# hermanjakobsen/robotic-ultrasound-imaging

Hardware: AMD Instinct MI355X
Metric: env-steps/sec (whole node) at 4096 envs/GPU, random-action rollout (higher is better)
Workload: dtype f32

## Files before the change

### robotic-ultrasound-imaging_amd/csrc/usim_step16.h

```cpp
#pragma once
#include <type_traits>

namespace usim {

template <int N, class F>
DI void static_for(F&& f) {
    if constexpr (N > 0) { static_for<N - 1>(f); f(std::integral_constant<int, N - 1>{}); }
}

template <int CTRL>
DI float dpp0(float v) { return __int_as_float(__builtin_amdgcn_update_dpp(0, __float_as_int(v), CTRL, 0xf, 0xf, true)); }
template <int G> DI int glane() { return (int)(threadIdx.x & (G - 1)); }
template <int G, int K> DI float rbc(float v) {
    if constexpr (G == 16) return dpp0<0x150 + K>(v);
    else {
        const int iv = __float_as_int(v);
        const int t = __builtin_amdgcn_update_dpp(iv, iv, 0x150 + K, 0xf, 0x3, false);
        return __int_as_float(__builtin_amdgcn_update_dpp(t, iv, 0x150 + 8 + K, 0xf, 0xc, false));
    }
}
template <int G, int D> DI float rshr0(float v) {
    const float t = dpp0<0x110 + D>(v);
    if constexpr (G == 16) return t; else return (glane<G>() < D) ? 0.f : t;
}
// ... 115 lines not shown
    P = mk(at[AT_LPOS], at[AT_LPOS + 1], at[AT_LPOS + 2]);
    static_for<3>([&](auto Dc) {
        constexpr int D = 1 << decltype(Dc)::value;
        const f3 LX = mk(rshr<G, D>(X.x, 1.f), rshr<G, D>(X.y, 0.f), rshr<G, D>(X.z, 0.f));
        const f3 LY = mk(rshr<G, D>(Y.x, 0.f), rshr<G, D>(Y.y, 1.f), rshr<G, D>(Y.z, 0.f));
        const f3 LZ = mk(rshr<G, D>(Z.x, 0.f), rshr<G, D>(Z.y, 0.f), rshr<G, D>(Z.z, 1.f));
        const f3 LP = mk(rshr0<G, D>(P.x), rshr0<G, D>(P.y), rshr0<G, D>(P.z));
        const f3 nX = LX * X.x + LY * X.y + LZ * X.z, nY = LX * Y.x + LY * Y.y + LZ * Y.z, nZ = LX * Z.x + LY * Z.y + LZ * Z.z;
        P = LP + LX * P.x + LY * P.y + LZ * P.z;
        X = nX; Y = nY; Z = nZ;
    });
}

DI void jacobian_rows(float* xl, const int gl, const float* Jc, float* Jr) {
    if (gl < 8) {
#pragma unroll
        for (int a = 0; a < 6; ++a) xl[a * 8 + gl] = Jc[a];
    }
    group_sync();
    int arow = (gl & 7) - ((gl & 4) ? 1 : 0);
    arow = arow > 5 ? 5 : arow;
    const float4 j0 = *reinterpret_cast<const float4*>(&xl[arow * 8]), j1 = *reinterpret_cast<const float4*>(&xl[arow * 8 + 4]);
    Jr[0] = j0.x; Jr[1] = j0.y; Jr[2] = j0.z; Jr[3] = j0.w; Jr[4] = j1.x; Jr[5] = j1.y; Jr[6] = j1.z; Jr[7] = j1.w;
}

template <int G>
DI float solve6_task(float* A, float b, const int gl) {
    static_for<6>([&](auto Kc) {
        constexpr int k = decltype(Kc)::value;
        constexpr int lk = TASK_LANE[k];
        const float g = (A[k] - (gl == lk ? 1.f : 0.f)) * rcp_(rbc<G, lk>(A[k]));
#pragma unroll
        for (int c = k + 1; c < 6; ++c) A[c] = fmaf(-g, rbc<G, lk>(A[c]), A[c]);
        b = fmaf(-g, rbc<G, lk>(b), b);
    });
    return b;
}

constexpr int X16_WORDS = 64;
constexpr int X16_RIGID_STRIDE = 84;

#ifndef USIM_WPR16
#define USIM_WPR16 4
#endif
#ifndef USIM_WPR8
#define USIM_WPR8 4
#endif
template <int G> constexpr int wpr() { return G == 16 ? USIM_WPR16 : USIM_WPR8; }
constexpr int MB_POSE = X16_WORDS;
constexpr int MB_OP = MB_POSE + 12;
constexpr int MB_W = MB_OP + 64;
constexpr int MB_Q = MB_W + 16;
constexpr int MB_GOAL = MB_Q + 100;
constexpr int X2_STRIDE = MB_GOAL + 12;
template <int G> constexpr int x2_base() { return TB_WORDS + (64 * wpr<G>() / G) * GE_STRIDE; }
static_assert(x2_base<16>() % 4 == 0 && x2_base<8>() % 4 == 0 && X2_STRIDE % 4 == 0 && MB_OP % 4 == 0 && MB_W % 4 == 0, "mailbox block: 16-byte accesses");
static_assert((x2_base<8>() + 32 * X2_STRIDE) * 4 <= 160 * 1024, "split kernel with 8-lane groups: LDS of a CU");
template <int G> constexpr int arm_cull_rounds() { return 7; }

#if defined(USIM_TSTAMP) || defined(USIM_TSTAMP_NOWAIT)
#define USIM_BAR() do { __syncthreads(); ++nbar; } while (0)
#else
#define USIM_BAR() __syncthreads()
#endif


constexpr int ARM_LDS_WORDS = A16_LANES * AT_STRIDE;
template <int TORSO, int ROLE, int G> constexpr int arm_lds_base();
template <int NE, class WR = NoWarm>
struct Carry {
    float dqj, qdj, q0j;
    Episode ep;
    float s[NE], sd[NE];
    WR wr;
};

template <int TORSO, int ROLE, int G> constexpr int arm_lds_base() {
    return ROLE != 0 ? x2_base<G>() + (64 * wpr<G>() / G) * X2_STRIDE : (TORSO ? SOFT16_LDS_WORDS : 16 * X16_RIGID_STRIDE);
}
static_assert((arm_lds_base<1, 1, 8>() + ARM_LDS_WORDS) * 4 <= 160 * 1024 && arm_lds_base<1, 1, 8>() % 4 == 0 && arm_lds_base<1, 1, 16>() % 4 == 0 && arm_lds_base<1, 0, 16>() % 4 == 0
              && arm_lds_base<0, 0, 16>() % 4 == 0, "arm table behind the LDS blocks of every 16-lane kernel");

template <int TORSO, int MODE, int ROLE, int NT, int G = 16, bool RES = false, class WR = NoWarm>
DI void step16_one(float* lds, const DevModel& M, const DevCfg& C, float* __restrict__ st, const int n, const int npad, const DevIO& io, const int flags, const long long rstep,
                   const bool first_pass, const int sub, int& nbar, Carry<TORSO ? (N_TOP + G - 1) / G : 1, WR>& cy) {
    constexpr bool WARM = !std::is_same<WR, NoWarm>::value;
    static_assert(!WARM || (TORSO == 1 && ROLE == 0) || (TORSO == 1 && MODE == 0), "warm start: the soft-torso kernels");
    constexpr int WPR = (ROLE != 0) ? wpr<G>() : 4;
    constexpr int EPW = 64 / G, EPB = WPR * EPW;
    static_assert(!RES || MODE == 0, "resident state: step launches only");
    constexpr int X2_BASE = x2_base<G>();
    constexpr unsigned GMASK = (G == 16) ? 0xffffu : 0xffu;
    static_assert(G == 16 || (TORSO == 1 && MODE == 0 && ROLE != 0), "8-lane groups: the split soft-torso step only");
    constexpr int NE = TORSO ? (N_TOP + G - 1) / G : 1;
    static_assert(ROLE == 0 || (TORSO == 1 && MODE == 0), "the split kernel is the soft-torso step");
    const int lane = threadIdx.x & 63, wave = (threadIdx.x >> 6) & (WPR - 1);
    constexpr bool RES_HERE = RES && !(ROLE == 2 && G == 16);
    const bool fresh = !RES_HERE || first_pass;
    const int gl = lane & (G - 1), ge = lane / G;
    const int gbase = lane - gl;
    const int eb = wave * EPW + ge;
    const bool auto_reset = (flags & LF_AUTO_RESET) != 0;
    unsigned long long* const dbg = io.dbg;
    const bool refill = (MODE == 1) && io.refill != 0;
    const int item_cnt = refill ? io.count[0] : 1;
    const int item_first = refill ? (int)blockIdx.x * EPB : 0;
    for (int item0 = item_first; item0 < item_cnt; item0 += refill ? (int)gridDim.x * EPB : 1) {
    int env = blockIdx.x * EPB + eb;
    bool valid = env < n;
    int item_ep = 0;
    if (refill) {
        valid = item0 + eb < item_cnt;
        const int2 it = valid ? io.items[item0 + eb] : make_int2(0, 0);
        env = it.x; item_ep = it.y;
    }
    const bool store = valid && gl == 0;
    const int ei = valid ? env : (refill ? 0 : n - 1);
#define LAT(w) st[(size_t)F_LAT * npad + (size_t)ei * LAT_ENV_WORDS + (w)]
#define EB(off) lds[TB_WORDS + eb * GE_STRIDE + (off)]
    float* const warm_rows = st + warm_index(io.bank_row0, npad, (size_t)ei);
    int mbo = X2_BASE + eb * X2_STRIDE;
    if constexpr (ROLE != 0) asm volatile("" : "+v"(mbo));
    float* const xl = (ROLE != 0) ? &lds[mbo]
                                  : (TORSO ? &lds[TB_WORDS + eb * GE_STRIDE + GE_WS] : &lds[eb * X16_RIGID_STRIDE]);
    static_assert(GE_WS + X16_WORDS <= GE_STRIDE, "transpose scratch overlays the wrench records");
    constexpr int GOAL_OFF = (ROLE != 0) ? MB_GOAL : (TORSO ? GE_CG + (MAXCAND + 1) * CG_WORDS - GE_WS : X16_WORDS);
    static_assert(GE_CG + (MAXCAND + 1) * CG_WORDS + 12 <= GE_STRIDE && X16_WORDS + 12 <= X16_RIGID_STRIDE, "room for the goal");
    float* const goal_lds = xl + GOAL_OFF;

    USIM_STAMP(dbg, 0);
    if constexpr (ROLE == 1) { if (dbg && blockIdx.x == 0 && threadIdx.x == 0) dbg[20] = __builtin_readcyclecounter(); }

    float at[AT_STRIDE];
    {
        constexpr int ARM_LDS = arm_lds_base<TORSO, ROLE, G>();
        const float4* ap = fresh ? reinterpret_cast<const float4*>(M.tables + TB_ARM + gl * AT_STRIDE) : reinterpret_cast<const float4*>(lds + ARM_LDS + gl * AT_STRIDE);
        if (fresh) {
#pragma unroll
            for (int v = 0; v < AT_STRIDE / 4; ++v) { const float4 x = ap[v]; at[4 * v] = x.x; at[4 * v + 1] = x.y; at[4 * v + 2] = x.z; at[4 * v + 3] = x.w; }
            if constexpr (RES && ROLE != 2) {
                if (lane < G) {
#pragma unroll
                    for (int v = 0; v < AT_STRIDE / 4; ++v) reinterpret_cast<float4*>(lds + ARM_LDS + gl * AT_STRIDE)[v] = make_float4(at[4 * v], at[4 * v + 1], at[4 * v + 2], at[4 * v + 3]);
// ... 58 lines not shown
        int tix = threadIdx.x;
        asm volatile("" : "+v"(tix));
#pragma unroll
        for (int i = 0; i < PER; ++i) { int idx = tix + i * NT; tmp[i] = (idx < NV) ? src[idx] : make_float4(0, 0, 0, 0); }
#pragma unroll
        for (int i = 0; i < PER; ++i) { int idx = tix + i * NT; if (idx < NV) dst[idx] = tmp[i]; }
        USIM_BAR();
    }
    USIM_STAMP(dbg, 1);

    if (MODE == 0 && sub == 0) t += 1;
    const bool last_sub = sub == C.substeps - 1;
    const int tphys = (MODE == 0) ? (t - 1) * C.substeps + sub : 0;
    const float dt = C.dt, inv_h = rcp_((float)C.horizon);
#if defined(USIM_TSTAMP) || defined(USIM_TSTAMP_NOWAIT)
#define RSTAMP(k) do { if (dbg && blockIdx.x == 0 && (threadIdx.x & (64 * WPR - 1)) == 0) dbg[(ROLE == 2 ? 30 : 20) + (k)] = __builtin_readcyclecounter(); } while (0)
#else
#define RSTAMP(k) do { } while (0)
#endif
#define XSTAMP(k) RSTAMP(20 + (k))
    if constexpr (ROLE == 2) {
        RSTAMP(0);
        float* const mb = &lds[mbo];
        const int* tb_shell = reinterpret_cast<const int*>(lds + TB_SHELL);
        float dz, vz, az;
        torso_motion(C, tphys, dz, vz, az);
        lattice_rhs<G, NE>(lds, eb, gl, M, az, kst, kdmp, true, s_pre, sd_pre);
        lattice_solve<G>(lds, eb, gl, gbase);
        RSTAMP(1);
        USIM_BAR();
        RSTAMP(2);
        const f3 xs = mk(mb[MB_POSE], mb[MB_POSE + 1], mb[MB_POSE + 2]), sy = mk(mb[MB_POSE + 3], mb[MB_POSE + 4], mb[MB_POSE + 5]),
                 sz = mk(mb[MB_POSE + 6], mb[MB_POSE + 7], mb[MB_POSE + 8]);
        const f3 sxc = cross(sy, sz);
        int nq = __float_as_int(mb[MB_POSE + 10]);
#pragma unroll
        for (int i = arm_cull_rounds<G>(); i < NE; ++i) {
            const int eraw = i * G + gl, e = eraw < N_TOP ? eraw : N_TOP - 1;
            const bool cand = (eraw < N_TOP) && collide_cull(lds, e, M, C, s_pre[i], dz, xs, sxc, sz);
            const unsigned gm = (unsigned)(__ballot(cand) >> gbase) & GMASK;
            mb[MB_Q + (cand ? nq + __popc(gm & ((1u << gl) - 1u)) : 99)] = __int_as_float(e);
            nq += __popc(gm);
        }
        group_sync();
        int nc = 0;
        collide_queue<G>(lds, mb + MB_Q, nq, &EB(GE_CG), gl, gbase, M, C, &EB(GE_S), dz, xs, sxc, sy, sz, nc);
        constexpr bool EARLY = G == 8;
        ContactRows P;
        int nc_early = nc, overflow_early = 0, ncmax_early = 0, cel_early[MAXC];
        if constexpr (EARLY) {
            contact_overflow<G>(lds, eb, gl, gbase, nc_early);
            if (nc_early > MAXC) { overflow_early = 1; nc_early = MAXC; }
            group_sync();
#pragma unroll
            for (int k = MAXC; k >= 1; --k) if (ncmax_early == 0 && __any(nc_early >= k)) ncmax_early = k;
#pragma unroll
            for (int k = 0; k < MAXC; ++k) cel_early[k] = (k < nc_early) ? __float_as_int(EB(GE_CG + k * CG_WORDS + 6)) : 0;
            if (ncmax_early > 0) contact_rows<G>(lds, eb, gl, M, C, nc_early, cel_early, vz, P);
        }
        RSTAMP(3);
        USIM_BAR();
        RSTAMP(4);
        if constexpr (!EARLY) contact_overflow<G>(lds, eb, gl, gbase, nc);
        int overflow = 0;
        if (nc > MAXC) { overflow = 1; nc = MAXC; }
        if constexpr (!EARLY) group_sync();
        XSTAMP(0);
        int ncmax = 0;
        if constexpr (EARLY) { nc = nc_early; overflow = overflow_early; ncmax = ncmax_early; }
        else {
#pragma unroll
            for (int k = MAXC; k >= 1; --k) if (ncmax == 0 && __any(nc >= k)) ncmax = k;
        }
        XSTAMP(1);
        float gf[MAXC], W[6] = {0, 0, 0, 0, 0, 0};
        int cel[MAXC];
#pragma unroll
        for (int k = 0; k < MAXC; ++k) { const int ek = __float_as_int(EB(GE_CG + k * CG_WORDS + 6)); gf[k] = 0.f; cel[k] = EARLY ? cel_early[k] : ((k < nc) ? ek : 0); }
        if (ncmax > 0) {
            float alpha[6], vs[6], Lp[21];
#pragma unroll
            for (int a = 0; a < 6; ++a) {
                alpha[a] = mb[MB_OP + 48 + a]; vs[a] = mb[MB_OP + 54 + a];
#pragma unroll
                for (int b = 0; b <= a; ++b) Lp[PK(a, b)] = mb[MB_OP + a * 8 + b];
            }
            XSTAMP(2);
            contact_solve<G, EARLY, true>(lds, eb, gl, M, C, nc, ncmax, cel, Lp, alpha, vs, mu, vz, P, W, gf, dbg, cy.wr);
            XSTAMP(3);
        } else warm_clear(cy.wr);
        if (gl == 0) {
            *reinterpret_cast<float4*>(&mb[MB_W]) = make_float4(W[0], W[1], W[2], W[3]);
            *reinterpret_cast<float4*>(&mb[MB_W + 4]) = make_float4(W[4], W[5], __int_as_float(nc), __int_as_float(overflow));
#pragma unroll
            for (int k = 0; k < MAXC; ++k) { const int sh = tb_shell[cel[k]]; mb[MB_W + 8 + k] = __int_as_float((k < nc) ? sh : -1); }
        }
        RSTAMP(5);
        USIM_BAR();
        RSTAMP(6);
        {
            float acc_e[NE];
#pragma unroll
            for (int i = 0; i < NE; ++i) { const int e = gl + i * G; acc_e[i] = (e < N_TOP) ? EB(GE_A + e) : 0.f; }
#pragma unroll
            for (int k = 0; k < MAXC; ++k) {
#pragma unroll
                for (int i = 0; i < NE; ++i) {
                    const int e = (gl + i * G < N_TOP) ? gl + i * G : N_TOP - 1;
                    acc_e[i] = fmaf(lds[TB_LINV + e * LROW + cel[k]], gf[k], acc_e[i]);
                }
            }
#pragma unroll
            for (int i = 0; i < NE; ++i) {
                const int e = gl + i * G;
                if (e >= N_TOP) continue;
                const float sdn = sd_pre[i] + dt * acc_e[i];
                const float sn = s_pre[i] + dt * sdn;
                if (valid) { LAT(LAT_SD + e) = sdn; LAT(LAT_S + e) = sn; }
                if constexpr (RES) { sd_pre[i] = sdn; s_pre[i] = sn; EB(GE_S + e) = sn; }
            }
            if constexpr (WARM) { if (valid) warm_store(warm_rows, gl, cy.wr); }
        }
        RSTAMP(7);
        USIM_BAR();
        RSTAMP(8);
        return;
// ... 60 lines not shown
            const f3 jv = cross(Z, xs - P);
            const float Jc[6] = {jlane ? jv.x : 0.f, jlane ? jv.y : 0.f, jlane ? jv.z : 0.f, jlane ? Z.x : 0.f, jlane ? Z.y : 0.f, jlane ? Z.z : 0.f};
            float Jr[8];
            jacobian_rows(xl, gl, Jc, Jr);
            float A6[6];
            static_for<6>([&](auto Bc) {
                constexpr int b = decltype(Bc)::value;
                float sacc = 0.f;
                static_for<NJ>([&](auto Jn) { constexpr int j = decltype(Jn)::value; sacc = fmaf(Jr[j], rbc<G, TASK_LANE[b]>(Jr[j]), sacc); });
                A6[b] = is_task ? sacc + ((gl == TASK_LANE[b]) ? 1e-6f : 0.f) : 0.f;
            });
            const float y = solve6_task<G>(A6, e, gl);
            const float dq = col_times_task<G>(Jc, y);
            qj = jlane ? qj + dq : 0.f;
            group_sync();
        }
        q0j = qj; qdj = 0.f; dqj = 0.f;
        episode_begin(E, 0);
    }

    f3 X, Y, Z, P;
    fk16<G>(at, qj, X, Y, Z, P);
    const f3 rcm = X * at[AT_LCOM] + Y * at[AT_LCOM + 1] + Z * at[AT_LCOM + 2];
    const f3 cm_ = P + rcm;
    const f3 sx = rbc3<G, 7>(X), sy = rbc3<G, 7>(Y), sz = rbc3<G, 7>(Z), xs = rbc3<G, 7>(P);
    const f3 hand = rbc3<G, NJ - 1>(P + X * M.hand7[0] + Y * M.hand7[1] + Z * M.hand7[2]);
    if constexpr (ROLE == 1) {
        {
            float dz_, vz_, az_;
            torso_motion(C, tphys, dz_, vz_, az_);
            const f3 sxc = cross(sy, sz);
            int nq = 0;
#pragma unroll
            for (int i = 0; i < NE; ++i) {
                const int eraw = i * G + gl, e = eraw < N_TOP ? eraw : N_TOP - 1;
                if (eraw < N_TOP) EB(GE_S + eraw) = s_pre[i];
                if (i >= arm_cull_rounds<G>()) continue;
                const bool cand = (eraw < N_TOP) && collide_cull(lds, e, M, C, s_pre[i], dz_, xs, sxc, sz);
                const unsigned gm = (unsigned)(__ballot(cand) >> gbase) & GMASK;
                xl[MB_Q + (cand ? nq + __popc(gm & ((1u << gl) - 1u)) : 99)] = __int_as_float(e);
                nq += __popc(gm);
            }
            if (gl == 0) xl[MB_POSE + 10] = __int_as_float(nq);
        }
        if (gl == 7) {
            float* mbp = xl + MB_POSE;
            mbp[0] = P.x; mbp[1] = P.y; mbp[2] = P.z; mbp[3] = Y.x; mbp[4] = Y.y; mbp[5] = Y.z; mbp[6] = Z.x; mbp[7] = Z.y; mbp[8] = Z.z;
        }
        if constexpr (ROLE == 1) RSTAMP(1);
        USIM_BAR();
        if constexpr (ROLE == 1) RSTAMP(2);
    }

    float act[7] = {0, 0, 0, 0, 0, 0, 0};
    if constexpr (MODE == 0) {
    if constexpr (ROLE != 2) {
    if (flags & LF_RANDOM_ACT) {
        const uint32_t gid = (uint32_t)(C.env_offset + ei);
        const u4 r = philox(gid, (uint32_t)rstep, (uint32_t)((unsigned long long)rstep >> 32), 1u + (uint32_t)(gl & 1), C.key0, C.key1);
        const float ra = __uint_as_float(r.a), rb = __uint_as_float(r.b), rc = __uint_as_float(r.c), rd = __uint_as_float(r.d);
        uint32_t rr[7];
        rr[0] = __float_as_uint(rbc<G, 0>(ra)); rr[1] = __float_as_uint(rbc<G, 0>(rb)); rr[2] = __float_as_uint(rbc<G, 0>(rc)); rr[3] = __float_as_uint(rbc<G, 0>(rd));
        rr[4] = __float_as_uint(rbc<G, 1>(ra)); rr[5] = __float_as_uint(rbc<G, 1>(rb)); rr[6] = __float_as_uint(rbc<G, 1>(rc));
#pragma unroll
        for (int a = 0; a < 7; ++a) {
            const float u = u01(rr[a]);
            const bool sgn = (C.mode == 1) || (C.mode == 3) || (C.mode == 2 && a == 6);
            act[a] = sgn ? 2.f * u - 1.f : u;
            if (C.mode == 3) act[a] *= WRENCH_MAX;
        }
        if (io.act_out && store) {
#pragma unroll
            for (int a = 0; a < 7; ++a) if (a < C.adim) io.act_out[(size_t)ei * C.adim + a] = act[a];
        }
    } else {
#pragma unroll
        for (int a = 0; a < 7; ++a) if (a < C.adim) act[a] = finite_or_zero(io.act[(size_t)ei * C.adim + a]);
    }
    }
    }
    float bias, Mr[NJ];
    f3 w, al, ao;
    {
        const f3 zq = Z * qdj;
        w = prefix_sum<G>(zq);
        const f3 wp = w - zq;
        const f3 dal = cross(wp, zq);
        al = prefix_sum<G>(dal);
        const f3 alp = al - dal;
        const f3 r = mk(P.x - rshr0<G, 1>(P.x), P.y - rshr0<G, 1>(P.y), P.z - rshr0<G, 1>(P.z));
        f3 da = cross(alp, r) + cross(wp, cross(wp, r));
        da.z += (gl == 0) ? GRAV : 0.f;
        ao = prefix_sum<G>(da);
        const f3 ac = ao + cross(al, rcm) + cross(w, cross(w, rcm));
        const float mass = at[AT_MASS];
        const f3 F = ac * mass;
        const float* I = &at[AT_INERTIA];
        const f3 RI0 = mk(X.x * I[0] + Y.x * I[1] + Z.x * I[2], X.x * I[1] + Y.x * I[3] + Z.x * I[4], X.x * I[2] + Y.x * I[4] + Z.x * I[5]);
        const f3 RI1 = mk(X.y * I[0] + Y.y * I[1] + Z.y * I[2], X.y * I[1] + Y.y * I[3] + Z.y * I[4], X.y * I[2] + Y.y * I[4] + Z.y * I[5]);
        const f3 RI2 = mk(X.z * I[0] + Y.z * I[1] + Z.z * I[2], X.z * I[1] + Y.z * I[3] + Z.z * I[4], X.z * I[2] + Y.z * I[4] + Z.z * I[5]);
        float Iw[6];
        Iw[0] = RI0.x * X.x + RI0.y * Y.x + RI0.z * Z.x; Iw[1] = RI0.x * X.y + RI0.y * Y.y + RI0.z * Z.y; Iw[2] = RI0.x * X.z + RI0.y * Y.z + RI0.z * Z.z;
        Iw[3] = RI1.x * X.y + RI1.y * Y.y + RI1.z * Z.y; Iw[4] = RI1.x * X.z + RI1.y * Y.z + RI1.z * Z.z; Iw[5] = RI2.x * X.z + RI2.y * Y.z + RI2.z * Z.z;
        const f3 Nc = symmul(Iw, al) + cross(w, symmul(Iw, w)) + cross(cm_, F);
        const f3 fa = suffix_sum<G>(F), na = suffix_sum<G>(Nc);
        bias = dot(Z, na - cross(P, fa));
        const float cc = dot(cm_, cm_);
        float Io[6] = {fmaf(mass, cc - cm_.x * cm_.x, Iw[0]), fmaf(-mass, cm_.x * cm_.y, Iw[1]), fmaf(-mass, cm_.x * cm_.z, Iw[2]),
                       fmaf(mass, cc - cm_.y * cm_.y, Iw[3]), fmaf(-mass, cm_.y * cm_.z, Iw[4]), fmaf(mass, cc - cm_.z * cm_.z, Iw[5])};
        const float cmass = suffix_sum<G>(mass);
        const f3 ch = suffix_sum<G>(cm_ * mass);
#pragma unroll
        for (int k = 0; k < 6; ++k) Io[k] = suffix_sum<G>(Io[k]);
        const f3 vo = cross(P, Z);
        const f3 nn = symmul(Io, Z) + cross(ch, vo);
        const f3 ff = vo * cmass + cross(Z, ch);
        float Ml[8];
        static_for<NJ>([&](auto Jc) {
            constexpr int j = decltype(Jc)::value;
            Ml[j] = spatial_dot_bc<G, j>(Z, vo, nn, ff);
        });
        Ml[7] = 0.f;
        if (gl < 8) {
// ... 125 lines not shown
    const float alpha_t = row_times_joint<G, NJ>(Jr, qs);
    f3 s_rc, s_wwrc, s_nw, s_arm, s_xso;
    float qe[4], obs[OBS_DIM], pos_err_norm = 0.f, pos_rew = 0.f, ori_err = 0.f, ori_rew = 0.f, vel_rew = 0.f, force_e = 0.f, dforce_e = 0.f;
    f3 xw, tpw;
    auto rot_inertia = [&](f3 v) {
        const f3 l = mk(dot(X, v), dot(Y, v), dot(Z, v));
        const f3 tt = symmul(M.pI7, l);
        return X * tt.x + Y * tt.y + Z * tt.z;
    };
    auto precompute = [&]() {
        s_rc = X * M.pcom7[0] + Y * M.pcom7[1] + Z * M.pcom7[2];
        s_wwrc = cross(w, cross(w, s_rc));
        s_nw = cross(w, rot_inertia(w));
        s_xso = xs - P;
        s_arm = s_rc - s_xso;
        const int tprev = (MODE == 0) ? t - 1 : 0;
        const float up = clampf((float)tprev * inv_h + u0, 0.f, 1.f);
        tpw = ts + (te - ts) * up;
        xw = mk(xs.x + M.base[0], xs.y + M.base[1], xs.z + M.base[2]);
        obs[12] = xw.x - tpw.x; obs[13] = xw.y - tpw.y; obs[14] = xw.z - tpw.z;
        mat2quat_xyzw(sx, sy, sz, qe);
        difference_quat(qe, M.gquat, obs + 15);
        if constexpr (MODE == 0) {
            float pe0 = 90.f * (xw.x - tpw.x), pe1 = 90.f * (xw.y - tpw.y);
            pe0 *= pe0; pe1 *= pe1;
            pos_err_norm = sqrt_(pe0 * pe0 + pe1 * pe1);
            pos_rew = 5.f * exp_(-pos_err_norm);
            const float qc[4] = {qe[3], qe[0], qe[1], qe[2]};
            ori_err = 0.2f * distance_quat_goal(qc, M.ghat, M.geps);
            ori_rew = exp_(-ori_err);
            float ve = 45.f * (vbar - 0.04f); ve *= ve;
            vel_rew = exp_(-ve);
            float fe = 0.7f * (fzbar - 5.f); fe *= fe;
            force_e = 3.f * exp_(-fe);
            float de = 0.01f * dfz; de *= de;
            dforce_e = 2.f * exp_(-de);
        }
    };
    float W[6] = {0, 0, 0, 0, 0, 0};
    int ncon = 0, overflow = 0, con_shell[MAXC];
#pragma unroll
    for (int k = 0; k < MAXC; ++k) con_shell[k] = -1;
    if constexpr (ROLE == 1) {
        if (is_task) {
            const int arow = blk ? 3 + comp : comp;
            float* mbo = xl + MB_OP;
            *reinterpret_cast<float4*>(&mbo[arow * 8]) = make_float4(Li[0], Li[1], Li[2], Li[3]);
            mbo[arow * 8 + 4] = Li[4]; mbo[arow * 8 + 5] = Li[5];
            mbo[48 + arow] = alpha_t; mbo[54 + arow] = v6;
        }
        RSTAMP(3);
        USIM_BAR();
        RSTAMP(4);
        precompute();
        RSTAMP(5);
        USIM_BAR();
        RSTAMP(6);
        const float4 w0 = *reinterpret_cast<const float4*>(&xl[MB_W]), w1 = *reinterpret_cast<const float4*>(&xl[MB_W + 4]);
        W[0] = w0.x; W[1] = w0.y; W[2] = w0.z; W[3] = w0.w; W[4] = w1.x; W[5] = w1.y;
        ncon = __float_as_int(w1.z); overflow = __float_as_int(w1.w);
#pragma unroll
        for (int k = 0; k < MAXC; ++k) con_shell[k] = __float_as_int(xl[MB_W + 8 + k]);
    } else if constexpr (TORSO != 0) {
        const int* tb_shell = reinterpret_cast<const int*>(lds + TB_SHELL);
        float dz, vz, az;
        torso_motion(C, tphys, dz, vz, az);
        lattice_rhs<G, NE>(lds, eb, gl, M, az, kst, kdmp, MODE == 0, s_pre, sd_pre);
        USIM_STAMP(dbg, 5);
        int nc = collide_all<G, NE>(lds, eb, gl, gbase, M, C, MODE == 0, s_pre, dz, xs, sy, sz);
        lattice_solve<G>(lds, eb, gl, gbase);
        contact_overflow<G>(lds, eb, gl, gbase, nc);
        USIM_STAMP(dbg, 7);
        if (nc > MAXC) { overflow = 1; nc = MAXC; }
        ncon = nc;
        group_sync();
        int ncmax = 0;
#pragma unroll
        for (int k = MAXC; k >= 1; --k) if (ncmax == 0 && __any(nc >= k)) ncmax = k;
        float gf[MAXC];
        int cel[MAXC];
#pragma unroll
        for (int k = 0; k < MAXC; ++k) { gf[k] = 0.f; cel[k] = (k < nc) ? __float_as_int(EB(GE_CG + k * CG_WORDS + 6)) : 0; }
        if (ncmax > 0) {
            float alpha[6], vs[6], Lp[21];
            static_for<6>([&](auto Ac) {
                constexpr int a = decltype(Ac)::value;
                alpha[a] = rbc<G, TASK_LANE[a]>(alpha_t); vs[a] = rbc<G, TASK_LANE[a]>(v6);
#pragma unroll
                for (int b = 0; b <= a; ++b) Lp[PK(a, b)] = rbc<G, TASK_LANE[a]>(Li[b]);
            });
            USIM_STAMP(dbg, 8);
            if constexpr (MODE == 0) contact_solve<G, false, false>(lds, eb, gl, M, C, nc, ncmax, cel, Lp, alpha, vs, mu, vz, ContactRows{}, W, gf, dbg, cy.wr);
            else { NoWarm cold; contact_solve<G, false, false>(lds, eb, gl, M, C, nc, ncmax, cel, Lp, alpha, vs, mu, vz, ContactRows{}, W, gf, dbg, cold); }
        } else warm_clear(cy.wr);
        USIM_STAMP(dbg, 11);
        if constexpr (MODE == 1) {
            if (valid && need && !refill) {
                for (int e = gl; e < N_TOP; e += G) { LAT(LAT_S + e) = 0.f; LAT(LAT_SD + e) = 0.f; }
                if constexpr (WARM) warm_rows_clear<G>(warm_rows, gl);
            }
        } else {
            float acc_e[NE];
#pragma unroll
            for (int i = 0; i < NE; ++i) { const int e = gl + i * G; acc_e[i] = (e < N_TOP) ? EB(GE_A + e) : 0.f; }
#pragma unroll
            for (int k = 0; k < MAXC; ++k) {
                if (k < ncmax) {
#pragma unroll
                    for (int i = 0; i < NE; ++i) {
                        const int e = (gl + i * G < N_TOP) ? gl + i * G : N_TOP - 1;
                        acc_e[i] = fmaf(lds[TB_LINV + e * LROW + cel[k]], gf[k], acc_e[i]);
                    }
                }
            }
#pragma unroll
            for (int i = 0; i < NE; ++i) {
                const int e = gl + i * G;
                if (e >= N_TOP) continue;
                const float sdn = sd_pre[i] + dt * acc_e[i];
                const float sn = s_pre[i] + dt * sdn;
                if (valid) { LAT(LAT_SD + e) = sdn; LAT(LAT_S + e) = sn; }
                if constexpr (RES) { sd_pre[i] = sdn; s_pre[i] = sn; }
            }
            if constexpr (WARM) { if (valid) warm_store(warm_rows, gl, cy.wr); }
        }
#pragma unroll
        for (int k = 0; k < MAXC; ++k) con_shell[k] = (k < nc) ? tb_shell[cel[k]] : -1;
    }
    USIM_STAMP(dbg, 12);

    if constexpr (ROLE != 1) precompute();
// ... 80 lines not shown
            if (jlane) L[26 + gl] = qj;
            if (gl == 0) {
                const float upn = clampf((float)t * inv_h + u0, 0.f, 1.f);
                const f3 tpn = ts + (te - ts) * upn;
                L[0] = xw.x; L[1] = xw.y; L[2] = xw.z; L[3] = tpn.x; L[4] = tpn.y; L[5] = tpn.z;
                L[6] = hv.x; L[7] = hv.y; L[8] = hv.z; L[9] = 0.04f; L[10] = vbar;
                L[11] = qe[0]; L[12] = qe[1]; L[13] = qe[2]; L[14] = qe[3];
                L[15] = M.gquat[0]; L[16] = M.gquat[1]; L[17] = M.gquat[2]; L[18] = M.gquat[3];
                L[19] = ori_err * 5.0f;
                L[20] = fz; L[21] = 5.0f; L[22] = fzbar; L[23] = dfz; L[24] = 0.f; L[25] = contact ? 1.f : 0.f;
                L[40] = (float)(t - 1) * inv_h * 100.f;
                L[41] = pos_rew; L[42] = ori_rew; L[43] = vel_rew; L[44] = force_rew; L[45] = dforce_rew;
            }
        }
        if (overflow) status |= 1;
        {
            const float chk = rbc<G, 7>(prefix_sum<G>(fabsf(qj) + 1e-3f * fabsf(qdj)));
            if (!(chk < 1.0e3f)) { status |= 4; done = true; epret -= reward; reward = 0.f; if (!(epret == epret)) epret = 0.f; }
        }
        if (store) {
            io.rew[ei] = reward;
            if (io.status_out) io.status_out[ei] = status;
            io.done[ei] = done ? 1 : 0;
            if (io.contacts) {
                io.contacts[(size_t)ei * (1 + MAXC)] = ncon;
#pragma unroll
                for (int k = 0; k < MAXC; ++k) io.contacts[(size_t)ei * (1 + MAXC) + 1 + k] = con_shell[k];
            }
            if (done) {
                if (io.term_obs) {
#pragma unroll
                    for (int a = 0; a < OBS_DIM; ++a) io.term_obs[(size_t)ei * OBS_DIM + a] = obs[a];
                }
                if (io.ep_ret) io.ep_ret[ei] = epret;
                if (io.ep_len) io.ep_len[ei] = t;
            }
        }
        need = done && auto_reset;
        if (store && io.obs && !need) {
#pragma unroll
            for (int a = 0; a < OBS_DIM; ++a) io.obs[(size_t)ei * OBS_DIM + a] = obs[a];
        }
        }
    }

    if constexpr (ROLE == 1) { RSTAMP(7); USIM_BAR(); RSTAMP(8); }
    if (MODE == 0 && need) {
        episode += 1;
        const int sl = episode & (BANK_DEPTH - 1);
        qj = jlane ? BK(sl, BQ0 + jl) : 0.f; q0j = qj; qdj = 0.f; dqj = 0.f;
        ts = mk(BK(sl, BTS), BK(sl, BTS + 1), BK(sl, BTS + 2)); te = mk(BK(sl, BTE), BK(sl, BTE + 1), BK(sl, BTE + 2));
        u0 = BK(sl, BU0); kst = BK(sl, BKST); kdmp = BK(sl, BKDMP); mu = BK(sl, BMU); fzbar = BK(sl, BFZ);
        episode_begin(E, BKI(sl, BSTATUS));
        if (store && io.obs) {
#pragma unroll
            for (int a = 0; a < OBS_DIM; ++a) io.obs[(size_t)ei * OBS_DIM + a] = BK(sl, BOBS + a);
        }
        if (TORSO && valid) for (int e = gl; e < N_TOP; e += G) { LAT(LAT_S + e) = 0.f; LAT(LAT_SD + e) = 0.f; }
        if constexpr (WARM) {
            if (valid) warm_rows_clear<G>(warm_rows, gl);
            warm_clear(cy.wr);
        }
        if constexpr (RES && TORSO != 0) {
#pragma unroll
            for (int i = 0; i < NE; ++i) {
                s_pre[i] = 0.f; sd_pre[i] = 0.f;
                if (ROLE == 1 && gl + i * G < N_TOP) EB(GE_S + gl + i * G) = 0.f;
            }
        }
        if (store) order_refill(io, env, episode);
    }
    if constexpr (RES && ROLE == 1) {
        if (gl == 0) *reinterpret_cast<float4*>(&xl[MB_W]) = make_float4(kst, kdmp, mu, (MODE == 0 && need) ? 1.f : 0.f);
    }
    USIM_STAMP(dbg, 15);

    if (valid && (MODE == 0 || (need && !refill))) {
        float* const so = st + scalar_index(0, (size_t)ei);
        if (jlane) {
            so[F_Q + gl] = dqj; so[F_QD + gl] = qdj;
            if (need) so[F_Q0 + gl] = q0j;
        }
        if (gl == 0) {
            float4* s4 = reinterpret_cast<float4*>(so);
            if (need) {
                so[F_TS] = ts.x; so[F_TS + 1] = ts.y; so[F_TS + 2] = ts.z;
                s4[6] = make_float4(te.x, te.y, te.z, u0);
            }
            s4[7] = make_float4(vbar, fzbar, fzprev, dfz);
            s4[8] = make_float4(kst, kdmp, mu, __int_as_float(t));
            s4[9] = make_float4(__int_as_float(touched), __int_as_float(episode), epret, __int_as_float(status));
        }
    }
    if (refill) group_sync();
    }
    if (MODE == 1 && refill) work_list_close(io);
    USIM_STAMP(dbg, 16);
    if constexpr (ROLE == 1) RSTAMP(9);
#undef RSTAMP
#undef XSTAMP
#undef LAT
#undef EB
}

template <int TORSO, int MODE, int ROLE, int NT, bool MULTI = false, int G = 16, class WR = NoWarm, bool ACTS = false>
DI void step16_body(float* lds, const DevModel& M, const DevCfg& C, float* __restrict__ st, const int n, const int npad, const DevIO& io0, const int flags, const long long rstep) {
    const int S = (MULTI && MODE == 0 && C.substeps > 1) ? C.substeps : 1;
    const int nsub = (MULTI && MODE == 0) ? (io0.nsub > 1 ? io0.nsub : 1) * S : 1;
    DevIO io = io0;
    int nbar = 0;
    Carry<TORSO ? (N_TOP + G - 1) / G : 1, WR> cy;
    int sub = 0;
    long long cstep = rstep;
    for (int ks = 0; ks < nsub; ++ks) {
        step16_one<TORSO, MODE, ROLE, NT, G, MULTI && MODE == 0, WR>(lds, M, C, st, n, npad, io, flags, cstep, ks == 0, sub, nbar, cy);
        const bool ctrl_done = sub == S - 1;
        if (ctrl_done) { sub = 0; ++cstep; } else ++sub;
        if (ks + 1 < nsub) {
            __threadfence_block();
            if constexpr (ROLE != 0) USIM_BAR();
            if (io0.block && ctrl_done) advance_rollout_block(io, (size_t)n, C.adim);
            if constexpr (ACTS) { if (ctrl_done) io.act += (size_t)n * C.adim; }
        }
    }
#if defined(USIM_TSTAMP) || defined(USIM_TSTAMP_NOWAIT)
    if (ROLE != 0 && io0.dbg && blockIdx.x == 0 && (threadIdx.x & (64 * wpr<G>() - 1)) == 0) io0.dbg[ROLE == 1 ? 46 : 47] = (unsigned long long)nbar;
#endif
}

template <int TORSO, int OCC, int MODE, bool MULTI = false, bool WARM = false>
__global__ __launch_bounds__(256) __attribute__((amdgpu_waves_per_eu(OCC, OCC))) void usim_step16_kernel(const DevModel M, const DevCfg C, float* __restrict__ st, int n, int npad,
                                                                                                          const DevIO io, int flags, long long rstep) {
    extern __shared__ __attribute__((aligned(16))) float lds[];
    step16_body<TORSO, MODE, 0, 256, MULTI, 16, typename std::conditional<WARM, WarmOf<16>::type, NoWarm>::type>(lds, M, C, st, n, npad, io, flags, rstep);
}

template <int TORSO, int OCC, bool WARM = false>
__global__ __launch_bounds__(256) __attribute__((amdgpu_waves_per_eu(OCC, OCC))) void usim_step16_acts_kernel(const DevModel M, const DevCfg C, float* __restrict__ st, int n, int npad,
                                                                                                               const DevIO io, int flags, long long rstep) {
    extern __shared__ __attribute__((aligned(16))) float lds[];
    step16_body<TORSO, 0, 0, 256, true, 16, typename std::conditional<WARM, WarmOf<16>::type, NoWarm>::type, true>(lds, M, C, st, n, npad, io, flags, rstep);
}

template <bool MULTI, int G = 16, bool WARM = false>
__global__ __launch_bounds__(128 * wpr<G>()) __attribute__((amdgpu_waves_per_eu(2, 2))) void usim_step32_kernel(const DevModel* __restrict__ Mp, const DevCfg* __restrict__ Cp, float* __restrict__ st, int n, int npad,
                                                                                                                  const DevIO io, int flags, long long rstep) {
    extern __shared__ __attribute__((aligned(16))) float lds[];
    const DevModel& M = *Mp; const DevCfg& C = *Cp;
    constexpr int NT = 128 * wpr<G>();
    typedef typename std::conditional<WARM, typename WarmOf<G>::type, NoWarm>::type WR;
    if (threadIdx.x < NT / 2) step16_body<1, 0, 1, NT, MULTI, G, WR>(lds, M, C, st, n, npad, io, flags, rstep);
    else step16_body<1, 0, 2, NT, MULTI, G, WR>(lds, M, C, st, n, npad, io, flags, rstep);
}

template <int G = 16, bool WARM = false>
__global__ __launch_bounds__(128 * wpr<G>()) __attribute__((amdgpu_waves_per_eu(2, 2))) void usim_step32_acts_kernel(const DevModel* __restrict__ Mp, const DevCfg* __restrict__ Cp, float* __restrict__ st, int n, int npad,
                                                                                                                       const DevIO io, int flags, long long rstep) {
    extern __shared__ __attribute__((aligned(16))) float lds[];
    const DevModel& M = *Mp; const DevCfg& C = *Cp;
    constexpr int NT = 128 * wpr<G>();
    typedef typename std::conditional<WARM, typename WarmOf<G>::type, NoWarm>::type WR;
    if (threadIdx.x < NT / 2) step16_body<1, 0, 1, NT, true, G, WR, true>(lds, M, C, st, n, npad, io, flags, rstep);
    else step16_body<1, 0, 2, NT, true, G, WR, true>(lds, M, C, st, n, npad, io, flags, rstep);
}

}
```

Before: 232.8 million.

## Draw next random action a pass ahead and reduce contact max via DPP

On the arm side of the split multi-step kernel, the philox random action for the next pass is drawn after a barrier and parked in a new per-env LDS mailbox slot. The following pass reads it back instead of regenerating it, taking the RNG off the critical path. Separately, the per-wave maximum contact count in the single (non-split) path now uses a DPP row-max reduction plus readlane instead of a loop of ballots. The mailbox stride grows by 8 words, which raises LDS use, and the parked action depends on the substep bookkeeping matching the caller's.

```diff
diff --git a/robotic-ultrasound-imaging_amd/csrc/usim_step16.h b/robotic-ultrasound-imaging_amd/csrc/usim_step16.h
--- a/robotic-ultrasound-imaging_amd/csrc/usim_step16.h
+++ b/robotic-ultrasound-imaging_amd/csrc/usim_step16.h
@@ -191,11 +191,32 @@
 constexpr int MB_W = MB_OP + 64;
 constexpr int MB_Q = MB_W + 16;
 constexpr int MB_GOAL = MB_Q + 100;
-constexpr int X2_STRIDE = MB_GOAL + 12;
+constexpr int MB_ACT = MB_GOAL + 12;
+constexpr int X2_STRIDE = MB_ACT + 8;
 template <int G> constexpr int x2_base() { return TB_WORDS + (64 * wpr<G>() / G) * GE_STRIDE; }
-static_assert(x2_base<16>() % 4 == 0 && x2_base<8>() % 4 == 0 && X2_STRIDE % 4 == 0 && MB_OP % 4 == 0 && MB_W % 4 == 0, "mailbox block: 16-byte accesses");
+static_assert(x2_base<16>() % 4 == 0 && x2_base<8>() % 4 == 0 && X2_STRIDE % 4 == 0 && MB_OP % 4 == 0 && MB_W % 4 == 0 && MB_ACT % 4 == 0, "mailbox block: 16-byte accesses");
 static_assert((x2_base<8>() + 32 * X2_STRIDE) * 4 <= 160 * 1024, "split kernel with 8-lane groups: LDS of a CU");
 template <int G> constexpr int arm_cull_rounds() { return 7; }
+
+constexpr bool ACT_PREFETCH = true;
+constexpr bool RESET_SETTLE = false;
+constexpr bool NCMAX_DPP_SPLIT = false, NCMAX_DPP_SINGLE = true;
+DI void settle_loads() { __builtin_amdgcn_s_waitcnt(0x0f70); }
+template <int G, bool DPP>
+DI int wave_ncmax(const int nc) {
+    if constexpr (DPP) {
+        int v = nc;
+        if constexpr (G == 8) v = max(v, __builtin_amdgcn_update_dpp(v, v, 0x128 , 0xf, 0xf, false));
+        v = max(v, __builtin_amdgcn_update_dpp(v, v, 0x142 , 0xa, 0xf, false));
+        v = max(v, __builtin_amdgcn_update_dpp(v, v, 0x143 , 0xc, 0xf, false));
+        return __builtin_amdgcn_readlane(v, 63);
+    } else {
+        int ncmax = 0;
+#pragma unroll
+        for (int k = MAXC; k >= 1; --k) if (ncmax == 0 && __any(nc >= k)) ncmax = k;
+        return ncmax;
+    }
+}
 
 #if defined(USIM_TSTAMP) || defined(USIM_TSTAMP_NOWAIT)
 #define USIM_BAR() do { __syncthreads(); ++nbar; } while (0)
@@ -220,7 +241,7 @@
 static_assert((arm_lds_base<1, 1, 8>() + ARM_LDS_WORDS) * 4 <= 160 * 1024 && arm_lds_base<1, 1, 8>() % 4 == 0 && arm_lds_base<1, 1, 16>() % 4 == 0 && arm_lds_base<1, 0, 16>() % 4 == 0
               && arm_lds_base<0, 0, 16>() % 4 == 0, "arm table behind the LDS blocks of every 16-lane kernel");
 
-template <int TORSO, int MODE, int ROLE, int NT, int G = 16, bool RES = false, class WR = NoWarm>
+template <int TORSO, int MODE, int ROLE, int NT, int G = 16, bool RES = false, class WR = NoWarm, bool PREACT = false>
 DI void step16_one(float* lds, const DevModel& M, const DevCfg& C, float* __restrict__ st, const int n, const int npad, const DevIO& io, const int flags, const long long rstep,
                    const bool first_pass, const int sub, int& nbar, Carry<TORSO ? (N_TOP + G - 1) / G : 1, WR>& cy) {
     constexpr bool WARM = !std::is_same<WR, NoWarm>::value;
@@ -228,6 +249,7 @@
     constexpr int WPR = (ROLE != 0) ? wpr<G>() : 4;
     constexpr int EPW = 64 / G, EPB = WPR * EPW;
     static_assert(!RES || MODE == 0, "resident state: step launches only");
+    static_assert(!PREACT || (RES && ROLE == 1), "action drawn a pass ahead: arm side of the split kernel, multi-step launches");
     constexpr int X2_BASE = x2_base<G>();
     constexpr unsigned GMASK = (G == 16) ? 0xffffu : 0xffu;
     static_assert(G == 16 || (TORSO == 1 && MODE == 0 && ROLE != 0), "8-lane groups: the split soft-torso step only");
@@ -392,8 +414,7 @@
             contact_overflow<G>(lds, eb, gl, gbase, nc_early);
             if (nc_early > MAXC) { overflow_early = 1; nc_early = MAXC; }
             group_sync();
-#pragma unroll
-            for (int k = MAXC; k >= 1; --k) if (ncmax_early == 0 && __any(nc_early >= k)) ncmax_early = k;
+            ncmax_early = wave_ncmax<G, NCMAX_DPP_SPLIT>(nc_early);
 #pragma unroll
             for (int k = 0; k < MAXC; ++k) cel_early[k] = (k < nc_early) ? __float_as_int(EB(GE_CG + k * CG_WORDS + 6)) : 0;
             if (ncmax_early > 0) contact_rows<G>(lds, eb, gl, M, C, nc_early, cel_early, vz, P);
@@ -408,10 +429,7 @@
         XSTAMP(0);
         int ncmax = 0;
         if constexpr (EARLY) { nc = nc_early; overflow = overflow_early; ncmax = ncmax_early; }
-        else {
-#pragma unroll
-            for (int k = MAXC; k >= 1; --k) if (ncmax == 0 && __any(nc >= k)) ncmax = k;
-        }
+        else ncmax = wave_ncmax<G, NCMAX_DPP_SPLIT>(nc);
         XSTAMP(1);
         float gf[MAXC], W[6] = {0, 0, 0, 0, 0, 0};
         int cel[MAXC];
@@ -578,23 +596,31 @@
         if constexpr (ROLE == 1) RSTAMP(2);
     }
 
+    auto draw_action = [&](const long long kstep, float* a7) {
+        const uint32_t gid = (uint32_t)(C.env_offset + ei);
+        const u4 r = philox(gid, (uint32_t)kstep, (uint32_t)((unsigned long long)kstep >> 32), 1u + (uint32_t)(gl & 1), C.key0, C.key1);
+        const float ra = __uint_as_float(r.a), rb = __uint_as_float(r.b), rc = __uint_as_float(r.c), rd = __uint_as_float(r.d);
+        uint32_t rr[7];
+        rr[0] = __float_as_uint(rbc<G, 0>(ra)); rr[1] = __float_as_uint(rbc<G, 0>(rb)); rr[2] = __float_as_uint(rbc<G, 0>(rc)); rr[3] = __float_as_uint(rbc<G, 0>(rd));
+        rr[4] = __float_as_uint(rbc<G, 1>(ra)); rr[5] = __float_as_uint(rbc<G, 1>(rb)); rr[6] = __float_as_uint(rbc<G, 1>(rc));
+#pragma unroll
+        for (int a = 0; a < 7; ++a) {
+            const float u = u01(rr[a]);
+            const bool sgn = (C.mode == 1) || (C.mode == 3) || (C.mode == 2 && a == 6);
+            a7[a] = sgn ? 2.f * u - 1.f : u;
+            if (C.mode == 3) a7[a] *= WRENCH_MAX;
+        }
+    };
     float act[7] = {0, 0, 0, 0, 0, 0, 0};
     if constexpr (MODE == 0) {
     if constexpr (ROLE != 2) {
     if (flags & LF_RANDOM_ACT) {
-        const uint32_t gid = (uint32_t)(C.env_offset + ei);
-        const u4 r = philox(gid, (uint32_t)rstep, (uint32_t)((unsigned long long)rstep >> 32), 1u + (uint32_t)(gl & 1), C.key0, C.key1);
-        const float ra = __uint_as_float(r.a), rb = __uint_as_float(r.b), rc = __uint_as_float(r.c), rd = __uint_as_float(r.d);
-        uint32_t rr[7];
-        rr[0] = __float_as_uint(rbc<G, 0>(ra)); rr[1] = __float_as_uint(rbc<G, 0>(rb)); rr[2] = __float_as_uint(rbc<G, 0>(rc)); rr[3] = __float_as_uint(rbc<G, 0>(rd));
-        rr[4] = __float_as_uint(rbc<G, 1>(ra)); rr[5] = __float_as_uint(rbc<G, 1>(rb)); rr[6] = __float_as_uint(rbc<G, 1>(rc));
-#pragma unroll
-        for (int a = 0; a < 7; ++a) {
-            const float u = u01(rr[a]);
-            const bool sgn = (C.mode == 1) || (C.mode == 3) || (C.mode == 2 && a == 6);
-            act[a] = sgn ? 2.f * u - 1.f : u;
-            if (C.mode == 3) act[a] *= WRENCH_MAX;
-        }
+        bool parked = false;
+        if constexpr (PREACT) parked = !first_pass;
+        if (parked) {
+            const float4 a0 = *reinterpret_cast<const float4*>(&xl[MB_ACT]), a1 = *reinterpret_cast<const float4*>(&xl[MB_ACT + 4]);
+            act[0] = a0.x; act[1] = a0.y; act[2] = a0.z; act[3] = a0.w; act[4] = a1.x; act[5] = a1.y; act[6] = a1.z;
+        } else draw_action(rstep, act);
         if (io.act_out && store) {
 #pragma unroll
             for (int a = 0; a < 7; ++a) if (a < C.adim) io.act_out[(size_t)ei * C.adim + a] = act[a];
@@ -826,6 +852,17 @@
         RSTAMP(3);
         USIM_BAR();
         RSTAMP(4);
+        if constexpr (PREACT) {
+            if (flags & LF_RANDOM_ACT) {
+                const bool ctrl_done = (C.substeps > 1) ? sub == C.substeps - 1 : true;
+                float nx[7];
+                draw_action(ctrl_done ? rstep + 1 : rstep, nx);
+                if (gl == 0) {
+                    *reinterpret_cast<float4*>(&xl[MB_ACT]) = make_float4(nx[0], nx[1], nx[2], nx[3]);
+                    *reinterpret_cast<float4*>(&xl[MB_ACT + 4]) = make_float4(nx[4], nx[5], nx[6], 0.f);
+                }
+            }
+        }
         precompute();
         RSTAMP(5);
         USIM_BAR();
@@ -848,9 +885,7 @@
         if (nc > MAXC) { overflow = 1; nc = MAXC; }
         ncon = nc;
         group_sync();
-        int ncmax = 0;
-#pragma unroll
-        for (int k = MAXC; k >= 1; --k) if (ncmax == 0 && __any(nc >= k)) ncmax = k;
+        const int ncmax = wave_ncmax<G, NCMAX_DPP_SINGLE>(nc);
         float gf[MAXC];
         int cel[MAXC];
 #pragma unroll
@@ -1037,6 +1072,7 @@
         ts = mk(BK(sl, BTS), BK(sl, BTS + 1), BK(sl, BTS + 2)); te = mk(BK(sl, BTE), BK(sl, BTE + 1), BK(sl, BTE + 2));
         u0 = BK(sl, BU0); kst = BK(sl, BKST); kdmp = BK(sl, BKDMP); mu = BK(sl, BMU); fzbar = BK(sl, BFZ);
         episode_begin(E, BKI(sl, BSTATUS));
+        if constexpr (RES && ROLE == 1 && RESET_SETTLE) settle_loads();
         if (store && io.obs) {
 #pragma unroll
             for (int a = 0; a < OBS_DIM; ++a) io.obs[(size_t)ei * OBS_DIM + a] = BK(sl, BOBS + a);
@@ -1098,7 +1134,7 @@
     int sub = 0;
     long long cstep = rstep;
     for (int ks = 0; ks < nsub; ++ks) {
-        step16_one<TORSO, MODE, ROLE, NT, G, MULTI && MODE == 0, WR>(lds, M, C, st, n, npad, io, flags, cstep, ks == 0, sub, nbar, cy);
+        step16_one<TORSO, MODE, ROLE, NT, G, MULTI && MODE == 0, WR, ACT_PREFETCH && MULTI && MODE == 0 && ROLE == 1 && !ACTS>(lds, M, C, st, n, npad, io, flags, cstep, ks == 0, sub, nbar, cy);
         const bool ctrl_done = sub == S - 1;
         if (ctrl_done) { sub = 0; ++cstep; } else ++sub;
         if (ks + 1 < nsub) {
```

Result: no change. 232.6 million (-0.1%).
